# InternRobotics/InternNav

Measured on NVIDIA H100. Metric: InternVLA-N1 policy-steps/sec (batch RGB-D+text->action), higher is better.
Workload: dtype bf16

## Files before the change

internnav_b200/_lib.py:

```python
import ctypes
import os
import threading

import torch

_HERE = os.path.dirname(os.path.abspath(__file__))
LIB_PATH = os.path.join(_HERE, "libn1b200.so")

_lib = None
_lock = threading.Lock()

c_void_p, c_int, c_size_t, c_float, c_char_p = (
    ctypes.c_void_p, ctypes.c_int, ctypes.c_size_t, ctypes.c_float, ctypes.c_char_p)


class N1Error(RuntimeError):
    def __init__(self, code, msg):
        super().__init__("n1b200 error %d: %s" % (code, msg))
        self.code = code


class TensorDesc(ctypes.Structure):
    _fields_ = [("name", c_char_p), ("data", c_void_p), ("dtype", ctypes.c_int32), ("ndim", ctypes.c_int32),
                ("shape", ctypes.c_int64 * 4)]
# ... 85 lines not shown
    assert t.is_cuda and t.is_contiguous(), "n1b200 takes contiguous CUDA tensors"
    return c_void_p(t.data_ptr())


def stream_ptr():
    return c_void_p(torch.cuda.current_stream().cuda_stream)


def dtype_code(t):
    if t.dtype == torch.float32:
        return 0
    if t.dtype == torch.bfloat16:
        return 1
    raise TypeError("n1b200 takes fp32 or bf16 tensors, got %s" % t.dtype)


def prof_enable(on):
    lib().n1_prof_enable(1 if on else 0)


def prof_read():
    a, b = ctypes.c_double(), ctypes.c_double()
    c, d = ctypes.c_int64(), ctypes.c_int64()
    check(lib().n1_prof_read(ctypes.byref(a), ctypes.byref(b), ctypes.byref(c), ctypes.byref(d)))
    return {"gemm_ms": a.value, "gemm_flops": b.value, "gemm_launches": c.value, "total_launches": d.value}


def prof_read_shapes(cap=256):
    mnk = (ctypes.c_int32 * (3 * cap))()
    cnt = (ctypes.c_int64 * cap)()
    ms = (ctypes.c_double * cap)()
    n = lib().n1_prof_read_shapes(mnk, cnt, ms, cap)
    if n < 0:
        raise N1Error(n, lib().n1_last_error().decode("utf-8", "replace"))
    return [dict(M=mnk[3 * i], N=mnk[3 * i + 1], K=mnk[3 * i + 2], count=int(cnt[i]), ms=float(ms[i])) for i in range(n)]


def gemm(a, w, bias=None, gamma=None, residual=None, act=ACT_NONE, out_fp32=False, out=None):
    assert a.dtype == torch.bfloat16 and w.dtype == torch.bfloat16 and a.dim() == 2 and w.dim() == 2
    M, K = a.shape
    N = w.shape[0]
    n_out = N // 2 if act == ACT_SWIGLU else N
    if out is None:
        out = torch.empty(M, n_out, device=a.device, dtype=torch.float32 if out_fp32 else torch.bfloat16)
    assert a.stride(1) == 1 and w.stride(1) == 1 and out.stride(1) == 1
    check(lib().n1_op_gemm(c_void_p(a.data_ptr()), a.stride(0), c_void_p(w.data_ptr()), w.stride(0),
                           c_void_p(out.data_ptr()), out.stride(0), M, N, K, ptr(bias), ptr(gamma),
                           c_void_p(residual.data_ptr()) if residual is not None else None,
                           residual.stride(0) if residual is not None else 0, act, 1 if out_fp32 else 0, stream_ptr()))
    return out


def gemm_tile(a, w, out, bias=None, gamma=None, residual=None, act=ACT_NONE, rows_per_group=0, group_stride=0,
              group_offset=0, row_add=None, tile_n=0):
    fn = lib().n1_test_gemm
    fn.restype = c_int
    fn.argtypes = [c_void_p, c_int, c_void_p, c_int, c_void_p, c_int, c_int, c_int, c_int, c_void_p, c_void_p, c_void_p,
                   c_int, c_int, c_int, c_int, c_int, c_int, c_void_p, c_int, c_void_p]
    vp = lambda t: c_void_p(t.data_ptr()) if t is not None else None
    check(fn(vp(a), a.stride(0), vp(w), w.stride(0), vp(out), out.stride(0), a.shape[0], w.shape[0], a.shape[1],
             vp(bias), vp(gamma), vp(residual), residual.stride(0) if residual is not None else 0, act,
             1 if out.dtype == torch.float32 else 0, rows_per_group, group_stride, group_offset, vp(row_add), tile_n,
             stream_ptr()))
    return out


def layernorm(x, w, b=None, eps=1e-5, rms=False, out=None):
    assert x.dtype == torch.bfloat16 and x.dim() == 2 and x.stride(1) == 1
    y = torch.empty(x.shape, device=x.device, dtype=torch.bfloat16) if out is None else out
    assert y.stride(1) == 1 and y.shape == x.shape
    check(lib().n1_op_layernorm(c_void_p(x.data_ptr()), x.stride(0), c_void_p(y.data_ptr()), y.stride(0), ptr(w), ptr(b), x.shape[0],
                                x.shape[1], eps, 1 if rms else 0, stream_ptr()))
    return y


MOD_RMS_SCALE, MOD_LN_SCALE, MOD_GATED_RESIDUAL = 0, 1, 2


def mod_norm(x, w, mod, rows_per_group, eps, mode, residual=None, out=None):
    assert x.dtype == torch.bfloat16 and x.dim() == 2 and x.stride(1) == 1
    if out is None:
        out = torch.empty(x.shape, device=x.device, dtype=torch.bfloat16)
    if mod is not None:
        assert mod.dtype == torch.bfloat16 and mod.stride(1) == 1 and mod.shape[1] == x.shape[1]
        assert mod.shape[0] * rows_per_group == x.shape[0]
    check(lib().n1_op_mod_norm(c_void_p(x.data_ptr()), x.stride(0), ptr(w), c_void_p(mod.data_ptr()) if mod is not None else None,
                               mod.stride(0) if mod is not None else 0, int(rows_per_group),
                               c_void_p(residual.data_ptr()) if residual is not None else None,
                               residual.stride(0) if residual is not None else 0, c_void_p(out.data_ptr()), out.stride(0),
                               x.shape[0], x.shape[1], float(eps), int(mode), stream_ptr()))
    return out


def add(a, b, out=None):
    assert a.dtype == torch.bfloat16 and b.dtype == torch.bfloat16 and a.is_contiguous() and b.is_contiguous() and a.shape == b.shape
    if out is None:
        out = torch.empty_like(a)
    check(lib().n1_op_add(ptr(a), ptr(b), ptr(out), a.numel(), stream_ptr()))
    return out


def action_embed(lat, w, b, pos, out=None):
    assert lat.dtype == torch.float32 and lat.is_contiguous() and lat.shape[-1] == 3
    rows, (T, D) = lat.numel() // 3, pos.shape
    if out is None:
        out = torch.empty(rows, D, device=lat.device, dtype=torch.bfloat16)
    check(lib().n1_op_action_embed(ptr(lat), ptr(w), ptr(b), ptr(pos), ptr(out), rows, T, D, stream_ptr()))
    return out


def cfg_euler(pred, n, cfg, scale, dt, lat):
    assert pred.dtype == torch.bfloat16 and pred.stride(1) == 1 and lat.dtype == torch.float32 and lat.is_contiguous()
    assert pred.shape[0] == (2 if cfg else 1) * n and lat.numel() == 3 * n
    check(lib().n1_op_cfg_euler(c_void_p(pred.data_ptr()), pred.stride(0), n, 1 if cfg else 0, float(scale), float(dt), ptr(lat),
                                stream_ptr()))
    return lat

# ... 65 lines not shown
```

internnav_b200/csrc/api.cu:

```cuda
#include <string.h>

#include <string>
#include <vector>

#include "../../include/n1b200.h"
#include "n1_ops.h"
#include "resize.h"
#include "bwd_kernels.h"
#include "s1_model.h"
#include "s2_kernels.h"
#include "s2_model.h"
#include "weights.h"

using namespace n1;

struct n1_ctx {
  int device = 0;
  S1Model s1;
  S2Model s2;
};
struct n1_vit_plan_s {
  VitPlan* p;
};
struct n1_llm_plan_s {
// ... 698 lines not shown
    if (cu) memcpy(cu, v.cu_window.data(), v.cu_window.size() * sizeof(int32_t));
    if (n_cu) *n_cu = (int32_t)v.cu_window.size();
    if (pos_hw) memcpy(pos_hw, v.pos_hw.data(), v.pos_hw.size() * sizeof(int32_t));
  });
}

void n1_prof_enable(int on) { prof_enable(on != 0); }

void n1_prof_add(int64_t gemm_launches, int64_t total_launches) {
  prof_count_launch((int)(total_launches - gemm_launches));
  for (int64_t i = 0; i < gemm_launches; ++i) prof_count_gemm(0.0);
}

int n1_prof_read_shapes(int32_t* mnk, int64_t* count, double* ms, int cap) {
  int n = -1;
  guard([&] {
    if (!mnk || !count || !ms || cap <= 0) throw Error(N1_ERR_ARG, "n1_prof_read_shapes: bad arguments");
    n = prof_read_shapes(mnk, reinterpret_cast<long*>(count), ms, cap);
  });
  return n;
}

int n1_prof_read(double* gemm_ms, double* gemm_flops, int64_t* gemm_launches, int64_t* total_launches) {
  return guard([&] {
    ProfStats st = prof_read_and_reset();
    if (gemm_ms) *gemm_ms = st.gemm_ms;
    if (gemm_flops) *gemm_flops = st.gemm_flops;
    if (gemm_launches) *gemm_launches = st.gemm_launches;
    if (total_launches) *total_launches = st.total_launches;
  });
}

int n1_op_gemm(const void* A, int lda, const void* W, int ldw, void* out, int ldo, int M, int N, int K,
               const float* bias, const float* gamma, const void* residual, int ldr, int act, int out_fp32,
               void* stream) {
  return guard([&] {
    GemmEpilogue e;
    e.bias = bias, e.gamma = gamma, e.residual = B16(residual), e.ldr = ldr, e.act = act, e.out_fp32 = out_fp32;
    gemm_bf16(B16(A), lda, B16(W), ldw, out, ldo, M, N, K, e, S(stream));
  });
}

int n1_test_gemm(const void* A, int lda, const void* W, int ldw, void* out, int ldo, int M, int N, int K, const float* bias,
                 const float* gamma, const void* residual, int ldr, int act, int out_fp32, int rows_per_group,
                 int group_stride, int group_offset, const float* row_add, int tile_n, void* stream) {
  return guard([&] {
    GemmEpilogue e;
    e.bias = bias, e.gamma = gamma, e.residual = B16(residual), e.ldr = ldr, e.act = act, e.out_fp32 = out_fp32;
    e.rows_per_group = rows_per_group, e.group_stride = group_stride, e.group_offset = group_offset, e.row_add = row_add;
    gemm_bf16(B16(A), lda, B16(W), ldw, out, ldo, M, N, K, e, S(stream), tile_n);
  });
}

int n1_op_ff_block(const void* x, int ldx, const float* ln_w, const float* ln_b, float eps, const void* w1, const float* b1,
                   const void* w2, const float* b2, void* out, int ldo, int M, void* stream) {
  return guard([&] {
    ff_block_384(B16(x), ldx, ln_w, ln_b, eps, B16(w1), b1, B16(w2), b2, B16(out), ldo, M, S(stream));
  });
}

int n1_op_dec_sa_block(void* x, int ldx, const float* ln_w, const float* ln_b, float eps, const void* w_qkv,
                       const float* b_qkv, const void* w_o, const float* b_o, int B, int Ns, int T, int causal, void* stream) {
  return guard([&] {
    dec_sa_block(B16(x), ldx, ln_w, ln_b, eps, B16(w_qkv), b_qkv, B16(w_o), b_o, B, Ns, T, causal, S(stream));
  });
}
int n1_op_dec_ca_block(void* x, int ldx, const float* ln_w, const float* ln_b, float eps, const void* w_q, const float* b_q,
                       const void* w_o, const float* b_o, const void* kv, int ldkv, int mtok, int B, int Ns, int T,
                       void* stream) {
  return guard([&] {
    dec_ca_block(B16(x), ldx, ln_w, ln_b, eps, B16(w_q), b_q, B16(w_o), b_o, B16(kv), ldkv, mtok, B, Ns, T, S(stream));
  });
}

int n1_op_mod_norm(const void* x, int ldx, const float* w, const void* mod, int ld_mod, int rows_per_group, const void* res,
                   int ldr, void* out, int ldo, int64_t rows, int D, float eps, int mode, void* stream) {
  return guard([&] {
    mod_norm(B16(x), ldx, w, B16(mod), ld_mod, rows_per_group, B16(res), ldr, B16(out), ldo, rows, D, eps, mode, S(stream));
  });
}
int n1_op_add(const void* a, const void* b, void* out, int64_t n, void* stream) {
  return guard([&] { add_bf16(B16(a), B16(b), B16(out), n, S(stream)); });
}
int n1_op_action_embed(const float* lat, const float* w, const float* b, const float* pos, void* out, int64_t rows, int T, int D,
                       void* stream) {
  return guard([&] { action_embed(lat, w, b, pos, B16(out), rows, T, D, S(stream)); });
}
int n1_op_cfg_euler(const void* pred, int ld, int64_t n, int cfg, float scale, float dt, float* lat, void* stream) {
  return guard([&] { cfg_euler(B16(pred), ld, n, cfg, scale, dt, lat, S(stream)); });
}
int n1_op_layernorm(const void* x, int ldx, void* y, int ldy, const float* w, const float* b, int rows, int D, float eps,
                    int rms, void* stream) {
  return guard([&] { layernorm(B16(x), ldx, B16(y), ldy, w, b, rows, D, eps, rms, S(stream)); });
}

int n1_op_attention(const void* q, const void* k, const void* v, void* o, int ldq, int ldk, int ldv, int ldo, int heads_q,
                    int heads_kv, int head_dim, int batch, int seq_q, int seq_k, const int32_t* cu_q,
                    const int32_t* cu_k, int max_seq_q, int kv_div, int causal, float scale, void* stream) {
  return guard([&] {
    AttnParams p = {};
    p.q = B16(q), p.k = B16(k), p.v = B16(v), p.o = B16(o);
    p.ldq = ldq, p.ldk = ldk, p.ldv = ldv, p.ldo = ldo;
    p.heads_q = heads_q, p.heads_kv = heads_kv, p.hd = head_dim, p.batch = batch;
    p.seq_q = seq_q, p.seq_k = seq_k, p.cu_q = cu_q, p.cu_k = cu_k, p.max_seq_q = max_seq_q;
    p.kv_div = kv_div < 1 ? 1 : kv_div, p.causal = causal, p.scale = scale;
    attention(p, S(stream));
// ... 33 lines not shown
```

internnav_b200/csrc/gemm_wgmma.cu:

```cuda
#include <stdlib.h>

#include <algorithm>
#include <atomic>
#include <mutex>
#include <vector>

#include "n1_ops.h"
#include "n1_ptx.cuh"

namespace n1 {

namespace {

constexpr int BM = 128;
constexpr int BK = 64;
constexpr int kConsumerWarps = 8;
constexpr int kThreads = 32 * kConsumerWarps + 128;

template <int BN>
struct Cfg {
  static constexpr int kABytes = BM * BK * 2;
  static constexpr int kBBytes = BN * BK * 2;
  static constexpr int kStageBytes = kABytes + kBBytes;
  static constexpr int kStages = BN == 256 ? 4 : BN == 128 ? 6 : 8;
  static constexpr int kBarBytes = 256;
  static constexpr int kStoreBytes = kConsumerWarps * 2 * 1024;
  static constexpr int kSmemBytes = kStages * kStageBytes + kBarBytes + kStoreBytes + 1024;
};
static_assert(Cfg<256>::kSmemBytes <= 232448 && Cfg<128>::kSmemBytes <= 232448 && Cfg<64>::kSmemBytes <= 232448,
              "GEMM shared memory budget (227 KB per block)");

constexpr long kWStreamsBytes = 32L << 20;

struct GemmArgs {
  int M, N, K;
  int tiles_m, tiles_n;
  void* out;
  int ldo;
  const float* bias;
  const float* gamma;
  const bf16* residual;
  int ldr;
  int act;
  int out_fp32;
  int rows_per_group, group_stride, group_offset;
  const float* row_add;
  int raster_g;
  int tma_store;
};

__device__ __forceinline__ void decode_tile(int tile, int tiles_m, int tiles_n, int G, int& tm, int& tn) {
  const int per_group = G * tiles_n;
  const int g = tile / per_group;
  const int first_m = g * G;
  const int gsize = min(G, tiles_m - first_m);
  const int r = tile - g * per_group;
  tm = first_m + r % gsize;
  tn = r / gsize;
}

__device__ __forceinline__ float apply_act(float v, int act) {
  if (act == ACT_GELU) return gelu_erf(v);
  if (act == ACT_RELU) return fmaxf(v, 0.0f);
  if (act == ACT_GELU_TANH)
    return 0.5f * v * (1.0f + tanhf(0.7978845608028654f * (v + 0.044715f * v * v * v)));
  if (act == ACT_SILU) return silu(v);
  return v;
}

template <int BN>
__global__ void __launch_bounds__(kThreads, 1)
gemm_kernel(const __grid_constant__ CUtensorMap tmA, const __grid_constant__ CUtensorMap tmB,
            const __grid_constant__ CUtensorMap tmC, const GemmArgs args) {
  using C = Cfg<BN>;
  extern __shared__ uint8_t smem_raw[];
  uint8_t* smem = reinterpret_cast<uint8_t*>((reinterpret_cast<uintptr_t>(smem_raw) + 1023) & ~uintptr_t(1023));
  uint8_t* sA = smem;
  uint8_t* sB = smem + C::kStages * C::kABytes;
  uint64_t* bars = reinterpret_cast<uint64_t*>(smem + C::kStages * C::kStageBytes);
  uint64_t* full = bars;
  uint64_t* empty = bars + C::kStages;
  uint8_t* sStore = smem + C::kStages * C::kStageBytes + C::kBarBytes;

  const int warp = threadIdx.x >> 5;
  const int lane = threadIdx.x & 31;
  const int num_tiles = args.tiles_m * args.tiles_n;
  const int nkb = (args.K + BK - 1) / BK;

  if (threadIdx.x == 0) {
    tma_prefetch_desc(&tmA);
    tma_prefetch_desc(&tmB);
    if (args.tma_store) tma_prefetch_desc(&tmC);
    for (int s = 0; s < C::kStages; ++s) {
      mbar_init(&full[s], 1);
      mbar_init(&empty[s], kConsumerWarps);
    }
    fence_mbar_init();
  }
  __syncthreads();

  if (warp >= kConsumerWarps) {
    setmaxnreg_dec<kProducerRegs>();
    if (warp == kConsumerWarps && lane == 0) {
      int stage = 0;
      uint32_t phase = 0;
      for (int tile = blockIdx.x; tile < num_tiles; tile += gridDim.x) {
        int tm, tn;
        decode_tile(tile, args.tiles_m, args.tiles_n, args.raster_g, tm, tn);
        for (int kb = 0; kb < nkb; ++kb) {
          mbar_wait(&empty[stage], phase ^ 1);
          mbar_arrive_expect_tx(&full[stage], C::kStageBytes);
          tma_load_2d(sA + stage * C::kABytes, &tmA, &full[stage], kb * BK, tm * BM);
          tma_load_2d(sB + stage * C::kBBytes, &tmB, &full[stage], kb * BK, tn * BN);
          if (++stage == C::kStages) {
            stage = 0;
            phase ^= 1;
          }
        }
      }
    }
  } else {
    setmaxnreg_inc<kConsumerRegs>();
    const int wg = warp >> 2;
    const int wrow = wg * 64 + (warp & 3) * 16;
    const int quad = lane & 3;
    const bool swiglu = args.act == ACT_SWIGLU;
    uint8_t* my_store = sStore + warp * 2048;
    int sbuf = 0;
    int stage = 0;
    uint32_t phase = 0;
    for (int tile = blockIdx.x; tile < num_tiles; tile += gridDim.x) {
      int tm, tn;
      decode_tile(tile, args.tiles_m, args.tiles_n, args.raster_g, tm, tn);
      float acc[BN / 2];
      int prev = -1;
      for (int kb = 0; kb < nkb; ++kb) {
        mbar_wait(&full[stage], phase);
        const uint64_t adesc = wgmma_desc_sw128(smem_u32(sA + stage * C::kABytes + wg * 64 * 128));
        const uint64_t bdesc = wgmma_desc_sw128(smem_u32(sB + stage * C::kBBytes));
        wgmma_fence();
#pragma unroll
        for (int k = 0; k < BK / 16; ++k)
          wgmma_ss<0, 0>(acc, adesc + 2 * k, bdesc + 2 * k, (kb | k) != 0 ? 1u : 0u);
        wgmma_commit();
        wgmma_wait<1>();
        if (prev >= 0 && lane == 0) mbar_arrive(&empty[prev]);
        prev = stage;
        if (++stage == C::kStages) {
          stage = 0;
          phase ^= 1;
        }
      }
      wgmma_wait<0>();
      if (prev >= 0 && lane == 0) mbar_arrive(&empty[prev]);

      int row[2];
      long out_row[2];
      int grp_row[2] = {0, 0};
      bool row_ok[2];
#pragma unroll
      for (int h = 0; h < 2; ++h) {
        row[h] = tm * BM + wrow + (lane >> 2) + h * 8;
        row_ok[h] = row[h] < args.M;
        out_row[h] = row[h];
        if (args.rows_per_group > 0) {
          grp_row[h] = row[h] % args.rows_per_group;
          out_row[h] = (long)(row[h] / args.rows_per_group) * args.group_stride + grp_row[h] + args.group_offset;
        }
      }
#pragma unroll
      for (int chunk = 0; chunk < BN / 32; ++chunk) {
        const int col0 = tn * BN + chunk * 32;
        if (col0 >= args.N) break;
        float v[4][4];
#pragma unroll
        for (int j = 0; j < 4; ++j) {
          const int col = col0 + j * 8 + quad * 2;
          const bool col_ok = col < args.N;
#pragma unroll
          for (int e = 0; e < 4; ++e) v[j][e] = acc[(chunk * 4 + j) * 4 + e];
          if (args.bias && col_ok) {
            const float2 b = __ldg(reinterpret_cast<const float2*>(args.bias + col));
            v[j][0] += b.x, v[j][1] += b.y, v[j][2] += b.x, v[j][3] += b.y;
          }
          if (swiglu) {
            v[j][0] = silu(v[j][0]) * v[j][1];
            v[j][2] = silu(v[j][2]) * v[j][3];
            continue;
          }
#pragma unroll
          for (int e = 0; e < 4; ++e) v[j][e] = apply_act(v[j][e], args.act);
          if (args.gamma && col_ok) {
            const float2 g = __ldg(reinterpret_cast<const float2*>(args.gamma + col));
            v[j][0] *= g.x, v[j][1] *= g.y, v[j][2] *= g.x, v[j][3] *= g.y;
          }
#pragma unroll
          for (int h = 0; h < 2; ++h) {
            if (!row_ok[h] || !col_ok) continue;
            if (args.row_add) {
              const float2 a = __ldg(reinterpret_cast<const float2*>(args.row_add + (long)grp_row[h] * args.N + col));
              v[j][2 * h] += a.x, v[j][2 * h + 1] += a.y;
            }
            if (args.residual) {
              const uint32_t q = __ldg(reinterpret_cast<const uint32_t*>(args.residual + out_row[h] * args.ldr + col));
              v[j][2 * h] += bf16_lo(q), v[j][2 * h + 1] += bf16_hi(q);
            }
          }
        }
        if (args.tma_store) {
          if (lane == 0) tma_store_wait_read<1>();
          __syncwarp();
          uint8_t* sb = my_store + sbuf * 1024;
#pragma unroll
          for (int j = 0; j < 4; ++j)
#pragma unroll
            for (int h = 0; h < 2; ++h) {
              const int r = (lane >> 2) + h * 8;
              if (swiglu)
                *reinterpret_cast<bf16*>(sb + r * 32 + (j * 4 + quad) * 2) = __float2bfloat16_rn(v[j][2 * h]);
              else
                *reinterpret_cast<uint32_t*>(sb + r * 64 + (j * 8 + quad * 2) * 2) = pack_bf16(v[j][2 * h], v[j][2 * h + 1]);
            }
          fence_proxy_async_smem();
          __syncwarp();
          if (lane == 0) {
            tma_store_2d(&tmC, sb, swiglu ? col0 >> 1 : col0, tm * BM + wrow);
            tma_store_commit();
          }
          sbuf ^= 1;
          continue;
        }
#pragma unroll
        for (int j = 0; j < 4; ++j) {
          const int col = col0 + j * 8 + quad * 2;
          if (col >= args.N) continue;
#pragma unroll
          for (int h = 0; h < 2; ++h) {
            if (!row_ok[h]) continue;
            if (swiglu)
              reinterpret_cast<bf16*>(args.out)[out_row[h] * args.ldo + (col >> 1)] = __float2bfloat16_rn(v[j][2 * h]);
            else if (args.out_fp32)
              *reinterpret_cast<float2*>(reinterpret_cast<float*>(args.out) + out_row[h] * args.ldo + col) =
                  make_float2(v[j][2 * h], v[j][2 * h + 1]);
            else
              *reinterpret_cast<uint32_t*>(reinterpret_cast<bf16*>(args.out) + out_row[h] * args.ldo + col) =
                  pack_bf16(v[j][2 * h], v[j][2 * h + 1]);
          }
        }
      }
    }
    if (args.tma_store && lane == 0) tma_store_wait<0>();
    __syncwarp();
  }
}

typedef CUresult (*EncodeTiledFn)(CUtensorMap*, CUtensorMapDataType, cuuint32_t, void*, const cuuint64_t*,
                                  const cuuint64_t*, const cuuint32_t*, const cuuint32_t*, CUtensorMapInterleave,
                                  CUtensorMapSwizzle, CUtensorMapL2promotion, CUtensorMapFloatOOBfill);

EncodeTiledFn encode_fn() {
  static EncodeTiledFn fn = nullptr;
  static std::once_flag once;
  std::call_once(once, [] {
    void* p = nullptr;
    cudaDriverEntryPointQueryResult q;
    cudaError_t e = cudaGetDriverEntryPoint("cuTensorMapEncodeTiled", &p, cudaEnableDefault, &q);
    if (e == cudaSuccess && q == cudaDriverEntryPointSuccess) fn = reinterpret_cast<EncodeTiledFn>(p);
  });
  if (!fn) throw Error(-4, "cuTensorMapEncodeTiled unavailable (no CUDA driver / GPU?)");
  return fn;
}

CUtensorMap make_map(const bf16* ptr, long rows, long cols, long ld, int box_rows, int box_cols = BK, bool swizzle = true) {
  N1_CHECK((reinterpret_cast<uintptr_t>(ptr) & 15) == 0, "GEMM operand not 16-byte aligned");
  N1_CHECK(ld % 8 == 0, "GEMM operand leading dimension must be a multiple of 8 elements");
  CUtensorMap m;
  cuuint64_t gdim[2] = {(cuuint64_t)cols, (cuuint64_t)rows};
  cuuint64_t gstr[1] = {(cuuint64_t)ld * 2};
  cuuint32_t box[2] = {(cuuint32_t)box_cols, (cuuint32_t)box_rows};
  cuuint32_t estr[2] = {1, 1};
  CUresult r = encode_fn()(&m, CU_TENSOR_MAP_DATA_TYPE_BFLOAT16, 2, const_cast<bf16*>(ptr), gdim, gstr, box, estr,
                           CU_TENSOR_MAP_INTERLEAVE_NONE, swizzle ? CU_TENSOR_MAP_SWIZZLE_128B : CU_TENSOR_MAP_SWIZZLE_NONE,
                           CU_TENSOR_MAP_L2_PROMOTION_L2_256B, CU_TENSOR_MAP_FLOAT_OOB_FILL_NONE);
  if (r != CUDA_SUCCESS) throw Error(-5, "cuTensorMapEncodeTiled failed: " + std::to_string((int)r));
  return m;
}

template <int BN>
void launch(const bf16* A, int lda, const bf16* W, int ldw, int M, int N, int K, GemmArgs& a, cudaStream_t stream) {
  using C = Cfg<BN>;
  static std::once_flag once;
  std::call_once(once, [] {
    cudaFuncSetAttribute(gemm_kernel<BN>, cudaFuncAttributeMaxDynamicSharedMemorySize, C::kSmemBytes);
  });
  a.tiles_m = (M + BM - 1) / BM;
  a.tiles_n = (N + BN - 1) / BN;
  {
    const long panel = (long)BM * K * 2;
    const long w_bytes = (long)N * K * 2;
    int g = 8;
    if (w_bytes > kWStreamsBytes) g = (int)std::max<long>(2, (16L << 20) / panel);
    a.raster_g = g < a.tiles_m ? g : a.tiles_m;
    if (a.raster_g < 1) a.raster_g = 1;
  }
  CUtensorMap tmA = make_map(A, M, K, lda, BM);
  CUtensorMap tmB = make_map(W, N, K, ldw, BN);
  CUtensorMap tmC = tmA;
  if (a.tma_store) {
    const bool sw = a.act == ACT_SWIGLU;
    tmC = make_map(static_cast<const bf16*>(a.out), M, sw ? N / 2 : N, a.ldo, 16, sw ? 16 : 32, false);
  }
  const int tiles = a.tiles_m * a.tiles_n;
  const int grid = tiles < device_sm_count() ? tiles : device_sm_count();
  gemm_kernel<BN><<<grid, kThreads, C::kSmemBytes, stream>>>(tmA, tmB, tmC, a);
  N1_CUDA(cudaGetLastError());
}

std::atomic<long> g_total_launches{0}, g_gemm_launches{0};
std::atomic<bool> g_prof_on{false};
std::mutex g_prof_mu;
struct EvPair {
  cudaEvent_t a, b;
  double flops;
  int M, N, K;
};
std::vector<EvPair> g_events;
struct ShapeAcc {
  int M, N, K;
  long count;
  double ms;
};
std::vector<ShapeAcc> g_shapes;

}

CUtensorMap tma_map_2d(const bf16* ptr, long rows, long cols, long ld, int box_rows, int box_cols, bool swizzle) {
  return make_map(ptr, rows, cols, ld, box_rows, box_cols, swizzle);
}
CUtensorMap tma_map_3d_sw128(const bf16* ptr, const long dims[3], const long strides[2], const int box[3]) {
  N1_CHECK((reinterpret_cast<uintptr_t>(ptr) & 15) == 0 && strides[0] % 8 == 0 && strides[1] % 8 == 0,
           "tma_map_3d_sw128: 16-byte alignment");
  CUtensorMap m;
  cuuint64_t gdim[3] = {(cuuint64_t)dims[0], (cuuint64_t)dims[1], (cuuint64_t)dims[2]};
  cuuint64_t gstr[2] = {(cuuint64_t)strides[0] * 2, (cuuint64_t)strides[1] * 2};
  cuuint32_t bx[3] = {(cuuint32_t)box[0], (cuuint32_t)box[1], (cuuint32_t)box[2]};
  cuuint32_t estr[3] = {1, 1, 1};
  CUresult r = encode_fn()(&m, CU_TENSOR_MAP_DATA_TYPE_BFLOAT16, 3, const_cast<bf16*>(ptr), gdim, gstr, bx, estr,
                           CU_TENSOR_MAP_INTERLEAVE_NONE, CU_TENSOR_MAP_SWIZZLE_128B, CU_TENSOR_MAP_L2_PROMOTION_L2_256B,
                           CU_TENSOR_MAP_FLOAT_OOB_FILL_NONE);
  if (r != CUDA_SUCCESS) throw Error(-5, "cuTensorMapEncodeTiled (3-D) failed: " + std::to_string((int)r));
  return m;
}
void prof_count_gemm(double flops) {
  (void)flops;
  g_gemm_launches++;
  g_total_launches++;
}

void prof_enable(bool on) { g_prof_on = on; }
int prof_begin(double flops, int M, int N, int K, cudaStream_t s) {
  if (!g_prof_on.load()) return -1;
  EvPair ev{};
  cudaEventCreate(&ev.a);
  cudaEventCreate(&ev.b);
  ev.flops = flops, ev.M = M, ev.N = N, ev.K = K;
  cudaEventRecord(ev.a, s);
  std::lock_guard<std::mutex> lk(g_prof_mu);
// ... 5 lines not shown
  std::lock_guard<std::mutex> lk(g_prof_mu);
  if (ticket < (int)g_events.size()) cudaEventRecord(g_events[ticket].b, s);
}
void prof_count_launch(int n) { g_total_launches += n; }
ProfStats prof_read_and_reset() {
  ProfStats st;
  std::lock_guard<std::mutex> lk(g_prof_mu);
  for (EvPair& e : g_events) {
    cudaEventSynchronize(e.b);
    float ms = 0.f;
    if (cudaEventElapsedTime(&ms, e.a, e.b) == cudaSuccess) {
      st.gemm_ms += ms, st.gemm_flops += e.flops;
      bool hit = false;
      for (ShapeAcc& sa : g_shapes)
        if (sa.M == e.M && sa.N == e.N && sa.K == e.K) {
          sa.count++, sa.ms += ms, hit = true;
          break;
        }
      if (!hit) g_shapes.push_back({e.M, e.N, e.K, 1, (double)ms});
    }
    cudaEventDestroy(e.a);
    cudaEventDestroy(e.b);
  }
  g_events.clear();
  st.gemm_launches = g_gemm_launches.exchange(0);
  st.total_launches = g_total_launches.exchange(0);
  return st;
}

int prof_read_shapes(int* mnk, long* count, double* ms, int cap) {
  std::lock_guard<std::mutex> lk(g_prof_mu);
  int n = 0;
  for (const ShapeAcc& sa : g_shapes) {
    if (n >= cap) break;
    mnk[3 * n] = sa.M, mnk[3 * n + 1] = sa.N, mnk[3 * n + 2] = sa.K;
    count[n] = sa.count, ms[n] = sa.ms;
    ++n;
  }
  g_shapes.clear();
  return n;
}

int device_sm_count() {
  static int sms = 0;
  if (!sms) {
    int dev = 0;
    cudaGetDevice(&dev);
    cudaDeviceGetAttribute(&sms, cudaDevAttrMultiProcessorCount, dev);
    if (sms <= 0) sms = 132;
  }
  return sms;
}

void gemm_bf16(const bf16* A, int lda, const bf16* W, int ldw, void* out, int ldo, int M, int N, int K,
               const GemmEpilogue& e, cudaStream_t stream, int tile_n) {
  if (M <= 0 || N <= 0) return;
  N1_CHECK(tile_n == 0 || tile_n == 64 || tile_n == 128 || tile_n == 256, "GEMM tile width must be 0, 64, 128 or 256");
  N1_CHECK(K > 0 && K % 8 == 0, "GEMM K must be a positive multiple of 8");
  N1_CHECK(N % 8 == 0, "GEMM N must be a multiple of 8 (pad the packed weight)");
  N1_CHECK(!(e.act == ACT_SWIGLU) || N % 16 == 0, "SwiGLU GEMM needs N % 16 == 0");
  GemmArgs a;
  a.M = M, a.N = N, a.K = K;
  a.out = out, a.ldo = ldo;
  a.bias = e.bias, a.gamma = e.gamma, a.residual = e.residual, a.ldr = e.ldr;
  a.act = e.act, a.out_fp32 = e.out_fp32;
  a.rows_per_group = e.rows_per_group, a.group_stride = e.group_stride, a.group_offset = e.group_offset;
  a.row_add = e.row_add;
  a.tma_store = (!e.out_fp32 && e.rows_per_group == 0 && (reinterpret_cast<uintptr_t>(out) & 15) == 0 && ldo % 8 == 0) ? 1 : 0;
  const int sms = device_sm_count();
  const int tm = (M + BM - 1) / BM;
  auto cost = [&](int bn) {
    const long tiles = (long)tm * ((N + bn - 1) / bn);
    const long waves = (tiles + sms - 1) / sms;
    return waves * (bn + 48);
  };
  int bn = tile_n;
  if (bn == 0) {
    bn = cost(128) <= cost(64) ? 128 : 64;
    if ((long)N * K * 2 > kWStreamsBytes && cost(256) <= cost(bn)) bn = 256;
  }
  const double flops = 2.0 * M * (double)N * K;
  const int ticket = prof_begin(flops, M, N, K, stream);
  prof_count_gemm(flops);
  if (bn == 256) launch<256>(A, lda, W, ldw, M, N, K, a, stream);
  else if (bn == 128) launch<128>(A, lda, W, ldw, M, N, K, a, stream);
  else launch<64>(A, lda, W, ldw, M, N, K, a, stream);
  prof_end(ticket, stream);
}

}
```

internnav_b200/csrc/n1_ops.h:

```cpp
#pragma once
#include <cuda.h>
#include <cuda_bf16.h>
#include <cuda_runtime.h>
#include <stdint.h>

#include <stdexcept>
#include <string>

namespace n1 {

typedef __nv_bfloat16 bf16;

struct Error : std::runtime_error {
  int code;
  Error(int c, const std::string& m) : std::runtime_error(m), code(c) {}
};

#define N1_CHECK(cond, msg)                                                                       \
  do {                                                                                            \
    if (!(cond)) throw ::n1::Error(-2, std::string(__FILE__) + ":" + std::to_string(__LINE__) + \
                                           ": " + (msg));                                         \
  } while (0)

#define N1_CUDA(call)                                                                              \
  do {                                                                                             \
    cudaError_t e__ = (call);                                                                      \
    if (e__ != cudaSuccess)                                                                        \
      throw ::n1::Error(-3, std::string(__FILE__) + ":" + std::to_string(__LINE__) + ": " + #call + \
                                ": " + cudaGetErrorString(e__));                                   \
  } while (0)

enum GemmAct { ACT_NONE = 0, ACT_GELU = 1, ACT_RELU = 2, ACT_SWIGLU = 3, ACT_GELU_TANH = 4, ACT_SILU = 5 };

struct GemmEpilogue {
  const float* bias = nullptr;
  const float* gamma = nullptr;
  const bf16* residual = nullptr;
  int ldr = 0;
  int act = ACT_NONE;
  int out_fp32 = 0;
  int rows_per_group = 0, group_stride = 0, group_offset = 0;
  const float* row_add = nullptr;
};

void gemm_bf16(const bf16* A, int lda, const bf16* W, int ldw, void* out, int ldo, int M, int N, int K,
               const GemmEpilogue& epi, cudaStream_t stream, int tile_n = 0);

int device_sm_count();

CUtensorMap tma_map_2d(const bf16* ptr, long rows, long cols, long ld, int box_rows, int box_cols, bool swizzle);
CUtensorMap tma_map_3d_sw128(const bf16* ptr, const long dims[3], const long strides[2], const int box[3]);
void prof_count_gemm(double flops);

struct ProfStats {
  double gemm_ms = 0, gemm_flops = 0;
  long gemm_launches = 0, total_launches = 0;
};
void prof_enable(bool on);
void prof_count_launch(int n = 1);
int prof_begin(double flops, int M, int N, int K, cudaStream_t s);
void prof_end(int ticket, cudaStream_t s);
ProfStats prof_read_and_reset();
int prof_read_shapes(int* mnk, long* count, double* ms, int cap);

void layernorm(const bf16* x, int ldx, bf16* y, int ldy, const float* w, const float* b, int rows, int D,
               float eps, int rms, cudaStream_t stream);

struct AttnParams {
  const bf16* q;
  const bf16* k;
  const bf16* v;
  bf16* o;
  int ldq, ldk, ldv, ldo;
  int heads_q, heads_kv, hd;
  int batch;
  int seq_q, seq_k;
  const int* cu_q;
  const int* cu_k;
  int kv_div;
  int causal;
  float scale;
  int max_seq_q;
  const int* k_len;
  int k_slot;
  long total_rows;
  const int* k_row0;
};
void attention(const AttnParams& p, cudaStream_t stream);
bool attention_tc_supported(const AttnParams& p);
bool attention_uses_tc(const AttnParams& p);
void attention_tc128(const AttnParams& p, cudaStream_t stream);

struct CacheAttnParams {
  const bf16* q;
  int ldq;
  long q_rows;
  const bf16 *k, *v;
  int ldkv;
  long kv_rows;
// ... 28 lines not shown
```

Before: 66.65.

## Add ping-pong warpgroup GEMM schedule for 128-wide tiles with multiple waves

Adds a ping-pong WGMMA kernel where the two consumer warpgroups take alternate 128x128 tiles, ordered by mbarriers, so one warpgroup's epilogue overlaps the other's MMA main loop. The heuristic selects it automatically when the 128-wide tile is chosen and the tile count exceeds the SM count. The producer and epilogue are factored into shared helpers, and the epilogue is rolled for the 128-register accumulator. The cost is higher register pressure per consumer and extra barrier handshakes between warpgroups.

```diff
diff --git a/internnav_b200/_lib.py b/internnav_b200/_lib.py
--- a/internnav_b200/_lib.py
+++ b/internnav_b200/_lib.py
@@ -161,17 +161,43 @@
 
 
 def gemm_tile(a, w, out, bias=None, gamma=None, residual=None, act=ACT_NONE, rows_per_group=0, group_stride=0,
-              group_offset=0, row_add=None, tile_n=0):
-    fn = lib().n1_test_gemm
+              group_offset=0, row_add=None, tile_n=0, schedule=None):
+    assert schedule in (None, "pingpong"), schedule
+    assert schedule is None or tile_n == 0, "the ping-pong schedule has one tile width"
+    vp = lambda t: c_void_p(t.data_ptr()) if t is not None else None
+    args = [vp(a), a.stride(0), vp(w), w.stride(0), vp(out), out.stride(0), a.shape[0], w.shape[0], a.shape[1],
+            vp(bias), vp(gamma), vp(residual), residual.stride(0) if residual is not None else 0, act,
+            1 if out.dtype == torch.float32 else 0, rows_per_group, group_stride, group_offset, vp(row_add)]
+    types = [c_void_p, c_int, c_void_p, c_int, c_void_p, c_int, c_int, c_int, c_int, c_void_p, c_void_p, c_void_p,
+             c_int, c_int, c_int, c_int, c_int, c_int, c_void_p]
+    if schedule == "pingpong":
+        fn = lib().n1_test_gemm_pingpong
+    else:
+        fn = lib().n1_test_gemm
+        args.append(tile_n)
+        types.append(c_int)
     fn.restype = c_int
-    fn.argtypes = [c_void_p, c_int, c_void_p, c_int, c_void_p, c_int, c_int, c_int, c_int, c_void_p, c_void_p, c_void_p,
-                   c_int, c_int, c_int, c_int, c_int, c_int, c_void_p, c_int, c_void_p]
-    vp = lambda t: c_void_p(t.data_ptr()) if t is not None else None
-    check(fn(vp(a), a.stride(0), vp(w), w.stride(0), vp(out), out.stride(0), a.shape[0], w.shape[0], a.shape[1],
-             vp(bias), vp(gamma), vp(residual), residual.stride(0) if residual is not None else 0, act,
-             1 if out.dtype == torch.float32 else 0, rows_per_group, group_stride, group_offset, vp(row_add), tile_n,
-             stream_ptr()))
-    return out
+    fn.argtypes = types + [c_void_p]
+    check(fn(*args, stream_ptr()))
+    return out
+
+
+def gemm_choice(M, N, K, sms):
+    fn = lib().n1_test_gemm_choice
+    fn.restype = c_int
+    fn.argtypes = [c_int, c_int, c_int, c_int, ctypes.POINTER(ctypes.c_int32), ctypes.POINTER(ctypes.c_int32)]
+    t, p = ctypes.c_int32(), ctypes.c_int32()
+    check(fn(M, N, K, sms, ctypes.byref(t), ctypes.byref(p)))
+    return t.value, bool(p.value)
+
+
+def gemm_pingpong_start(wg, j, cta, grid, nkb):
+    fn = lib().n1_test_gemm_pingpong_start
+    fn.restype = c_int
+    fn.argtypes = [c_int, c_int, c_int, c_int, c_int, ctypes.POINTER(ctypes.c_int32)]
+    out = (ctypes.c_int32 * 4)()
+    check(fn(wg, j, cta, grid, nkb, out))
+    return tuple(out)
 
 
 def layernorm(x, w, b=None, eps=1e-5, rms=False, out=None):
diff --git a/internnav_b200/csrc/api.cu b/internnav_b200/csrc/api.cu
--- a/internnav_b200/csrc/api.cu
+++ b/internnav_b200/csrc/api.cu
@@ -774,6 +774,34 @@
   });
 }
 
+int n1_test_gemm_pingpong(const void* A, int lda, const void* W, int ldw, void* out, int ldo, int M, int N, int K,
+                          const float* bias, const float* gamma, const void* residual, int ldr, int act, int out_fp32,
+                          int rows_per_group, int group_stride, int group_offset, const float* row_add, void* stream) {
+  return guard([&] {
+    GemmEpilogue e;
+    e.bias = bias, e.gamma = gamma, e.residual = B16(residual), e.ldr = ldr, e.act = act, e.out_fp32 = out_fp32;
+    e.rows_per_group = rows_per_group, e.group_stride = group_stride, e.group_offset = group_offset, e.row_add = row_add;
+    gemm_bf16(B16(A), lda, B16(W), ldw, out, ldo, M, N, K, e, S(stream), 0, true);
+  });
+}
+int n1_test_gemm_choice(int M, int N, int K, int sms, int32_t* tile_n, int32_t* pingpong) {
+  return guard([&] {
+    if (M <= 0 || N <= 0 || K <= 0 || sms <= 0 || !tile_n || !pingpong)
+      throw Error(N1_ERR_ARG, "n1_test_gemm_choice: bad arguments");
+    const GemmChoice c = gemm_choice(M, N, K, sms);
+    *tile_n = c.tile_n, *pingpong = c.pingpong ? 1 : 0;
+  });
+}
+int n1_test_gemm_pingpong_start(int wg, int j, int cta, int grid, int nkb, int32_t* out4) {
+  return guard([&] {
+    if (wg < 0 || wg > 1 || j < 0 || cta < 0 || grid <= cta || nkb <= 0 || !out4)
+      throw Error(N1_ERR_ARG, "n1_test_gemm_pingpong_start: bad arguments");
+    const int stages = gemm_pingpong_stages();
+    const PingPongStart st = pingpong_start(wg, j, cta, grid, nkb, stages);
+    out4[0] = st.tile, out4[1] = st.stage, out4[2] = (int32_t)st.phase, out4[3] = stages;
+  });
+}
+
 int n1_op_ff_block(const void* x, int ldx, const float* ln_w, const float* ln_b, float eps, const void* w1, const float* b1,
                    const void* w2, const float* b2, void* out, int ldo, int M, void* stream) {
   return guard([&] {
diff --git a/internnav_b200/csrc/gemm_wgmma.cu b/internnav_b200/csrc/gemm_wgmma.cu
--- a/internnav_b200/csrc/gemm_wgmma.cu
+++ b/internnav_b200/csrc/gemm_wgmma.cu
@@ -27,6 +27,7 @@
   static constexpr int kStoreBytes = kConsumerWarps * 2 * 1024;
   static constexpr int kSmemBytes = kStages * kStageBytes + kBarBytes + kStoreBytes + 1024;
 };
+static_assert(2 * Cfg<128>::kStages + 2 <= Cfg<128>::kBarBytes / 8, "ping-pong barriers: full, empty, order");
 static_assert(Cfg<256>::kSmemBytes <= 232448 && Cfg<128>::kSmemBytes <= 232448 && Cfg<64>::kSmemBytes <= 232448,
               "GEMM shared memory budget (227 KB per block)");
 
@@ -69,6 +70,148 @@
 }
 
 template <int BN>
+__device__ __forceinline__ void produce(const CUtensorMap* tmA, const CUtensorMap* tmB, const GemmArgs& args, uint8_t* sA,
+                                        uint8_t* sB, uint64_t* full, uint64_t* empty, int num_tiles, int nkb) {
+  using C = Cfg<BN>;
+  int stage = 0;
+  uint32_t phase = 0;
+  for (int tile = blockIdx.x; tile < num_tiles; tile += gridDim.x) {
+    int tm, tn;
+    decode_tile(tile, args.tiles_m, args.tiles_n, args.raster_g, tm, tn);
+    for (int kb = 0; kb < nkb; ++kb) {
+      mbar_wait(&empty[stage], phase ^ 1);
+      mbar_arrive_expect_tx(&full[stage], C::kStageBytes);
+      tma_load_2d(sA + stage * C::kABytes, tmA, &full[stage], kb * BK, tm * BM);
+      tma_load_2d(sB + stage * C::kBBytes, tmB, &full[stage], kb * BK, tn * BN);
+      if (++stage == C::kStages) {
+        stage = 0;
+        phase ^= 1;
+      }
+    }
+  }
+}
+
+__device__ __forceinline__ void epilogue_chunk(const float* a, const GemmArgs& args, const CUtensorMap* tmC, int tm,
+                                               int col0, int wrow, int lane, uint8_t* my_store, int& sbuf) {
+  const int quad = lane & 3;
+  const bool swiglu = args.act == ACT_SWIGLU;
+  int row[2];
+  long out_row[2];
+  int grp_row[2] = {0, 0};
+  bool row_ok[2];
+#pragma unroll
+  for (int h = 0; h < 2; ++h) {
+    row[h] = tm * BM + wrow + (lane >> 2) + h * 8;
+    row_ok[h] = row[h] < args.M;
+    out_row[h] = row[h];
+    if (args.rows_per_group > 0) {
+      grp_row[h] = row[h] % args.rows_per_group;
+      out_row[h] = (long)(row[h] / args.rows_per_group) * args.group_stride + grp_row[h] + args.group_offset;
+    }
+  }
+  {
+    float v[4][4];
+#pragma unroll
+    for (int j = 0; j < 4; ++j) {
+      const int col = col0 + j * 8 + quad * 2;
+      const bool col_ok = col < args.N;
+#pragma unroll
+      for (int e = 0; e < 4; ++e) v[j][e] = a[j * 4 + e];
+      if (args.bias && col_ok) {
+        const float2 b = __ldg(reinterpret_cast<const float2*>(args.bias + col));
+        v[j][0] += b.x, v[j][1] += b.y, v[j][2] += b.x, v[j][3] += b.y;
+      }
+      if (swiglu) {
+        v[j][0] = silu(v[j][0]) * v[j][1];
+        v[j][2] = silu(v[j][2]) * v[j][3];
+        continue;
+      }
+#pragma unroll
+      for (int e = 0; e < 4; ++e) v[j][e] = apply_act(v[j][e], args.act);
+      if (args.gamma && col_ok) {
+        const float2 g = __ldg(reinterpret_cast<const float2*>(args.gamma + col));
+        v[j][0] *= g.x, v[j][1] *= g.y, v[j][2] *= g.x, v[j][3] *= g.y;
+      }
+#pragma unroll
+      for (int h = 0; h < 2; ++h) {
+        if (!row_ok[h] || !col_ok) continue;
+        if (args.row_add) {
+          const float2 a = __ldg(reinterpret_cast<const float2*>(args.row_add + (long)grp_row[h] * args.N + col));
+          v[j][2 * h] += a.x, v[j][2 * h + 1] += a.y;
+        }
+        if (args.residual) {
+          const uint32_t q = __ldg(reinterpret_cast<const uint32_t*>(args.residual + out_row[h] * args.ldr + col));
+          v[j][2 * h] += bf16_lo(q), v[j][2 * h + 1] += bf16_hi(q);
+        }
+      }
+    }
+    if (args.tma_store) {
+      if (lane == 0) tma_store_wait_read<1>();
+      __syncwarp();
+      uint8_t* sb = my_store + sbuf * 1024;
+#pragma unroll
+      for (int j = 0; j < 4; ++j)
+#pragma unroll
+        for (int h = 0; h < 2; ++h) {
+          const int r = (lane >> 2) + h * 8;
+          if (swiglu)
+            *reinterpret_cast<bf16*>(sb + r * 32 + (j * 4 + quad) * 2) = __float2bfloat16_rn(v[j][2 * h]);
+          else
+            *reinterpret_cast<uint32_t*>(sb + r * 64 + (j * 8 + quad * 2) * 2) = pack_bf16(v[j][2 * h], v[j][2 * h + 1]);
+        }
+      fence_proxy_async_smem();
+      __syncwarp();
+      if (lane == 0) {
+        tma_store_2d(tmC, sb, swiglu ? col0 >> 1 : col0, tm * BM + wrow);
+        tma_store_commit();
+      }
+      sbuf ^= 1;
+      return;
+    }
+#pragma unroll
+    for (int j = 0; j < 4; ++j) {
+      const int col = col0 + j * 8 + quad * 2;
+      if (col >= args.N) continue;
+#pragma unroll
+      for (int h = 0; h < 2; ++h) {
+        if (!row_ok[h]) continue;
+        if (swiglu)
+          reinterpret_cast<bf16*>(args.out)[out_row[h] * args.ldo + (col >> 1)] = __float2bfloat16_rn(v[j][2 * h]);
+        else if (args.out_fp32)
+          *reinterpret_cast<float2*>(reinterpret_cast<float*>(args.out) + out_row[h] * args.ldo + col) =
+              make_float2(v[j][2 * h], v[j][2 * h + 1]);
+        else
+          *reinterpret_cast<uint32_t*>(reinterpret_cast<bf16*>(args.out) + out_row[h] * args.ldo + col) =
+              pack_bf16(v[j][2 * h], v[j][2 * h + 1]);
+      }
+    }
+  }
+}
+
+
+template <int NV, int BN, bool kRolled>
+__device__ __forceinline__ void epilogue(float (&acc)[NV], const GemmArgs& args, const CUtensorMap* tmC, int tm, int tn,
+                                         int wrow, int lane, uint8_t* my_store, int& sbuf) {
+  constexpr int kPerSlab = BN / 32;
+  if constexpr (kRolled) {
+#pragma unroll 1
+    for (int c = 0; c < NV / 16; ++c) {
+      const int col0 = tn * BN + (c % kPerSlab) * 32;
+      if (col0 < args.N)
+        epilogue_chunk(acc, args, tmC, tm, col0, wrow + (c / kPerSlab) * 64, lane, my_store, sbuf);
+#pragma unroll
+      for (int i = 0; i + 16 < NV; ++i) acc[i] = acc[i + 16];
+    }
+  } else {
+#pragma unroll
+    for (int c = 0; c < NV / 16; ++c) {
+      const int col0 = tn * BN + (c % kPerSlab) * 32;
+      if (col0 < args.N) epilogue_chunk(acc + 16 * c, args, tmC, tm, col0, wrow + (c / kPerSlab) * 64, lane, my_store, sbuf);
+    }
+  }
+}
+
+template <int BN>
 __global__ void __launch_bounds__(kThreads, 1)
 gemm_kernel(const __grid_constant__ CUtensorMap tmA, const __grid_constant__ CUtensorMap tmB,
             const __grid_constant__ CUtensorMap tmC, const GemmArgs args) {
@@ -101,30 +244,10 @@
 
   if (warp >= kConsumerWarps) {
     setmaxnreg_dec<kProducerRegs>();
-    if (warp == kConsumerWarps && lane == 0) {
-      int stage = 0;
-      uint32_t phase = 0;
-      for (int tile = blockIdx.x; tile < num_tiles; tile += gridDim.x) {
-        int tm, tn;
-        decode_tile(tile, args.tiles_m, args.tiles_n, args.raster_g, tm, tn);
-        for (int kb = 0; kb < nkb; ++kb) {
-          mbar_wait(&empty[stage], phase ^ 1);
-          mbar_arrive_expect_tx(&full[stage], C::kStageBytes);
-          tma_load_2d(sA + stage * C::kABytes, &tmA, &full[stage], kb * BK, tm * BM);
-          tma_load_2d(sB + stage * C::kBBytes, &tmB, &full[stage], kb * BK, tn * BN);
-          if (++stage == C::kStages) {
-            stage = 0;
-            phase ^= 1;
-          }
-        }
-      }
-    }
+    if (warp == kConsumerWarps && lane == 0) produce<BN>(&tmA, &tmB, args, sA, sB, full, empty, num_tiles, nkb);
   } else {
     setmaxnreg_inc<kConsumerRegs>();
     const int wg = warp >> 2;
-    const int wrow = wg * 64 + (warp & 3) * 16;
-    const int quad = lane & 3;
-    const bool swiglu = args.act == ACT_SWIGLU;
     uint8_t* my_store = sStore + warp * 2048;
     int sbuf = 0;
     int stage = 0;
@@ -153,101 +276,91 @@
       }
       wgmma_wait<0>();
       if (prev >= 0 && lane == 0) mbar_arrive(&empty[prev]);
-
-      int row[2];
-      long out_row[2];
-      int grp_row[2] = {0, 0};
-      bool row_ok[2];
-#pragma unroll
-      for (int h = 0; h < 2; ++h) {
-        row[h] = tm * BM + wrow + (lane >> 2) + h * 8;
-        row_ok[h] = row[h] < args.M;
-        out_row[h] = row[h];
-        if (args.rows_per_group > 0) {
-          grp_row[h] = row[h] % args.rows_per_group;
-          out_row[h] = (long)(row[h] / args.rows_per_group) * args.group_stride + grp_row[h] + args.group_offset;
-        }
-      }
-#pragma unroll
-      for (int chunk = 0; chunk < BN / 32; ++chunk) {
-        const int col0 = tn * BN + chunk * 32;
-        if (col0 >= args.N) break;
-        float v[4][4];
-#pragma unroll
-        for (int j = 0; j < 4; ++j) {
-          const int col = col0 + j * 8 + quad * 2;
-          const bool col_ok = col < args.N;
-#pragma unroll
-          for (int e = 0; e < 4; ++e) v[j][e] = acc[(chunk * 4 + j) * 4 + e];
-          if (args.bias && col_ok) {
-            const float2 b = __ldg(reinterpret_cast<const float2*>(args.bias + col));
-            v[j][0] += b.x, v[j][1] += b.y, v[j][2] += b.x, v[j][3] += b.y;
-          }
-          if (swiglu) {
-            v[j][0] = silu(v[j][0]) * v[j][1];
-            v[j][2] = silu(v[j][2]) * v[j][3];
-            continue;
-          }
-#pragma unroll
-          for (int e = 0; e < 4; ++e) v[j][e] = apply_act(v[j][e], args.act);
-          if (args.gamma && col_ok) {
-            const float2 g = __ldg(reinterpret_cast<const float2*>(args.gamma + col));
-            v[j][0] *= g.x, v[j][1] *= g.y, v[j][2] *= g.x, v[j][3] *= g.y;
-          }
-#pragma unroll
-          for (int h = 0; h < 2; ++h) {
-            if (!row_ok[h] || !col_ok) continue;
-            if (args.row_add) {
-              const float2 a = __ldg(reinterpret_cast<const float2*>(args.row_add + (long)grp_row[h] * args.N + col));
-              v[j][2 * h] += a.x, v[j][2 * h + 1] += a.y;
-            }
-            if (args.residual) {
-              const uint32_t q = __ldg(reinterpret_cast<const uint32_t*>(args.residual + out_row[h] * args.ldr + col));
-              v[j][2 * h] += bf16_lo(q), v[j][2 * h + 1] += bf16_hi(q);
-            }
-          }
-        }
-        if (args.tma_store) {
-          if (lane == 0) tma_store_wait_read<1>();
-          __syncwarp();
-          uint8_t* sb = my_store + sbuf * 1024;
-#pragma unroll
-          for (int j = 0; j < 4; ++j)
-#pragma unroll
-            for (int h = 0; h < 2; ++h) {
-              const int r = (lane >> 2) + h * 8;
-              if (swiglu)
-                *reinterpret_cast<bf16*>(sb + r * 32 + (j * 4 + quad) * 2) = __float2bfloat16_rn(v[j][2 * h]);
-              else
-                *reinterpret_cast<uint32_t*>(sb + r * 64 + (j * 8 + quad * 2) * 2) = pack_bf16(v[j][2 * h], v[j][2 * h + 1]);
-            }
-          fence_proxy_async_smem();
-          __syncwarp();
-          if (lane == 0) {
-            tma_store_2d(&tmC, sb, swiglu ? col0 >> 1 : col0, tm * BM + wrow);
-            tma_store_commit();
-          }
-          sbuf ^= 1;
-          continue;
-        }
-#pragma unroll
-        for (int j = 0; j < 4; ++j) {
-          const int col = col0 + j * 8 + quad * 2;
-          if (col >= args.N) continue;
-#pragma unroll
-          for (int h = 0; h < 2; ++h) {
-            if (!row_ok[h]) continue;
-            if (swiglu)
-              reinterpret_cast<bf16*>(args.out)[out_row[h] * args.ldo + (col >> 1)] = __float2bfloat16_rn(v[j][2 * h]);
-            else if (args.out_fp32)
-              *reinterpret_cast<float2*>(reinterpret_cast<float*>(args.out) + out_row[h] * args.ldo + col) =
-                  make_float2(v[j][2 * h], v[j][2 * h + 1]);
-            else
-              *reinterpret_cast<uint32_t*>(reinterpret_cast<bf16*>(args.out) + out_row[h] * args.ldo + col) =
-                  pack_bf16(v[j][2 * h], v[j][2 * h + 1]);
-          }
-        }
-      }
+      epilogue<BN / 2, BN, false>(acc, args, &tmC, tm, tn, wg * 64 + (warp & 3) * 16, lane, my_store, sbuf);
+    }
+    if (args.tma_store && lane == 0) tma_store_wait<0>();
+    __syncwarp();
+  }
+}
+
+__global__ void __launch_bounds__(kThreads, 1)
+gemm_pingpong(const __grid_constant__ CUtensorMap tmA, const __grid_constant__ CUtensorMap tmB,
+              const __grid_constant__ CUtensorMap tmC, const GemmArgs args) {
+  using C = Cfg<128>;
+  extern __shared__ uint8_t smem_raw[];
+  uint8_t* smem = reinterpret_cast<uint8_t*>((reinterpret_cast<uintptr_t>(smem_raw) + 1023) & ~uintptr_t(1023));
+  uint8_t* sA = smem;
+  uint8_t* sB = smem + C::kStages * C::kABytes;
+  uint64_t* bars = reinterpret_cast<uint64_t*>(smem + C::kStages * C::kStageBytes);
+  uint64_t* full = bars;
+  uint64_t* empty = bars + C::kStages;
+  uint64_t* order = bars + 2 * C::kStages;
+  uint8_t* sStore = smem + C::kStages * C::kStageBytes + C::kBarBytes;
+
+  const int warp = threadIdx.x >> 5;
+  const int lane = threadIdx.x & 31;
+  const int num_tiles = args.tiles_m * args.tiles_n;
+  const int nkb = (args.K + BK - 1) / BK;
+
+  if (threadIdx.x == 0) {
+    tma_prefetch_desc(&tmA);
+    tma_prefetch_desc(&tmB);
+    if (args.tma_store) tma_prefetch_desc(&tmC);
+    for (int s = 0; s < C::kStages; ++s) {
+      mbar_init(&full[s], 1);
+      mbar_init(&empty[s], kConsumerWarps / 2);
+    }
+    mbar_init(&order[0], kConsumerWarps / 2);
+    mbar_init(&order[1], kConsumerWarps / 2);
+    fence_mbar_init();
+  }
+  __syncthreads();
+
+  if (warp >= kConsumerWarps) {
+    setmaxnreg_dec<kProducerRegs>();
+    if (warp == kConsumerWarps && lane == 0) produce<128>(&tmA, &tmB, args, sA, sB, full, empty, num_tiles, nkb);
+  } else {
+    setmaxnreg_inc<kConsumerRegs>();
+    const int wg = warp >> 2;
+    uint8_t* my_store = sStore + warp * 2048;
+    int sbuf = 0;
+    for (int j = 0;; ++j) {
+      const PingPongStart st = pingpong_start(wg, j, blockIdx.x, gridDim.x, nkb, C::kStages);
+      if (st.tile >= num_tiles) break;
+      int tm, tn;
+      decode_tile(st.tile, args.tiles_m, args.tiles_n, args.raster_g, tm, tn);
+      if (wg == 1) mbar_wait(&order[0], j & 1);
+      else if (j > 0) mbar_wait(&order[1], (j - 1) & 1);
+      int stage = st.stage;
+      uint32_t phase = st.phase;
+      float acc[128];
+      float(&acc_lo)[64] = *reinterpret_cast<float(*)[64]>(acc);
+      float(&acc_hi)[64] = *reinterpret_cast<float(*)[64]>(acc + 64);
+      int prev = -1;
+      for (int kb = 0; kb < nkb; ++kb) {
+        mbar_wait(&full[stage], phase);
+        const uint64_t adesc0 = wgmma_desc_sw128(smem_u32(sA + stage * C::kABytes));
+        const uint64_t adesc1 = wgmma_desc_sw128(smem_u32(sA + stage * C::kABytes + 64 * 128));
+        const uint64_t bdesc = wgmma_desc_sw128(smem_u32(sB + stage * C::kBBytes));
+        wgmma_fence();
+#pragma unroll
+        for (int k = 0; k < BK / 16; ++k) {
+          wgmma_ss<0, 0>(acc_lo, adesc0 + 2 * k, bdesc + 2 * k, (kb | k) != 0 ? 1u : 0u);
+          wgmma_ss<0, 0>(acc_hi, adesc1 + 2 * k, bdesc + 2 * k, (kb | k) != 0 ? 1u : 0u);
+        }
+        wgmma_commit();
+        wgmma_wait<1>();
+        if (prev >= 0 && lane == 0) mbar_arrive(&empty[prev]);
+        prev = stage;
+        if (++stage == C::kStages) {
+          stage = 0;
+          phase ^= 1;
+        }
+      }
+      if (lane == 0) mbar_arrive(&order[wg]);
+      wgmma_wait<0>();
+      if (lane == 0) mbar_arrive(&empty[prev]);
+      epilogue<128, 128, true>(acc, args, &tmC, tm, tn, (warp & 3) * 16, lane, my_store, sbuf);
     }
     if (args.tma_store && lane == 0) tma_store_wait<0>();
     __syncwarp();
@@ -286,12 +399,14 @@
   return m;
 }
 
-template <int BN>
+template <int BN, bool kPingPong>
 void launch(const bf16* A, int lda, const bf16* W, int ldw, int M, int N, int K, GemmArgs& a, cudaStream_t stream) {
   using C = Cfg<BN>;
+  static_assert(!kPingPong || BN == 128, "the ping-pong schedule has 128 x 128 tiles");
+  const auto kernel = kPingPong ? gemm_pingpong : gemm_kernel<BN>;
   static std::once_flag once;
-  std::call_once(once, [] {
-    cudaFuncSetAttribute(gemm_kernel<BN>, cudaFuncAttributeMaxDynamicSharedMemorySize, C::kSmemBytes);
+  std::call_once(once, [kernel] {
+    cudaFuncSetAttribute(kernel, cudaFuncAttributeMaxDynamicSharedMemorySize, C::kSmemBytes);
   });
   a.tiles_m = (M + BM - 1) / BM;
   a.tiles_n = (N + BN - 1) / BN;
@@ -312,7 +427,7 @@
   }
   const int tiles = a.tiles_m * a.tiles_n;
   const int grid = tiles < device_sm_count() ? tiles : device_sm_count();
-  gemm_kernel<BN><<<grid, kThreads, C::kSmemBytes, stream>>>(tmA, tmB, tmC, a);
+  kernel<<<grid, kThreads, C::kSmemBytes, stream>>>(tmA, tmB, tmC, a);
   N1_CUDA(cudaGetLastError());
 }
 
@@ -424,10 +539,24 @@
   return sms;
 }
 
+int gemm_pingpong_stages() { return Cfg<128>::kStages; }
+
+GemmChoice gemm_choice(int M, int N, int K, int sms) {
+  const int tm = (M + BM - 1) / BM;
+  auto tiles = [&](int bn) { return (long)tm * ((N + bn - 1) / bn); };
+  auto cost = [&](int bn) { return (tiles(bn) + sms - 1) / sms * (bn + 48); };
+  GemmChoice c;
+  c.tile_n = cost(128) <= cost(64) ? 128 : 64;
+  if ((long)N * K * 2 > kWStreamsBytes && cost(256) <= cost(c.tile_n)) c.tile_n = 256;
+  c.pingpong = c.tile_n == 128 && tiles(128) > sms;
+  return c;
+}
+
 void gemm_bf16(const bf16* A, int lda, const bf16* W, int ldw, void* out, int ldo, int M, int N, int K,
-               const GemmEpilogue& e, cudaStream_t stream, int tile_n) {
+               const GemmEpilogue& e, cudaStream_t stream, int tile_n, bool pingpong) {
   if (M <= 0 || N <= 0) return;
   N1_CHECK(tile_n == 0 || tile_n == 64 || tile_n == 128 || tile_n == 256, "GEMM tile width must be 0, 64, 128 or 256");
+  N1_CHECK(!pingpong || tile_n == 0, "the ping-pong GEMM schedule has one tile width; pass tile_n = 0");
   N1_CHECK(K > 0 && K % 8 == 0, "GEMM K must be a positive multiple of 8");
   N1_CHECK(N % 8 == 0, "GEMM N must be a multiple of 8 (pad the packed weight)");
   N1_CHECK(!(e.act == ACT_SWIGLU) || N % 16 == 0, "SwiGLU GEMM needs N % 16 == 0");
@@ -439,24 +568,16 @@
   a.rows_per_group = e.rows_per_group, a.group_stride = e.group_stride, a.group_offset = e.group_offset;
   a.row_add = e.row_add;
   a.tma_store = (!e.out_fp32 && e.rows_per_group == 0 && (reinterpret_cast<uintptr_t>(out) & 15) == 0 && ldo % 8 == 0) ? 1 : 0;
-  const int sms = device_sm_count();
-  const int tm = (M + BM - 1) / BM;
-  auto cost = [&](int bn) {
-    const long tiles = (long)tm * ((N + bn - 1) / bn);
-    const long waves = (tiles + sms - 1) / sms;
-    return waves * (bn + 48);
-  };
-  int bn = tile_n;
-  if (bn == 0) {
-    bn = cost(128) <= cost(64) ? 128 : 64;
-    if ((long)N * K * 2 > kWStreamsBytes && cost(256) <= cost(bn)) bn = 256;
-  }
+  GemmChoice c{tile_n, pingpong};
+  if (tile_n == 0 && !pingpong) c = gemm_choice(M, N, K, device_sm_count());
+  if (c.pingpong) c.tile_n = 128;
   const double flops = 2.0 * M * (double)N * K;
   const int ticket = prof_begin(flops, M, N, K, stream);
   prof_count_gemm(flops);
-  if (bn == 256) launch<256>(A, lda, W, ldw, M, N, K, a, stream);
-  else if (bn == 128) launch<128>(A, lda, W, ldw, M, N, K, a, stream);
-  else launch<64>(A, lda, W, ldw, M, N, K, a, stream);
+  if (c.pingpong) launch<128, true>(A, lda, W, ldw, M, N, K, a, stream);
+  else if (c.tile_n == 256) launch<256, false>(A, lda, W, ldw, M, N, K, a, stream);
+  else if (c.tile_n == 128) launch<128, false>(A, lda, W, ldw, M, N, K, a, stream);
+  else launch<64, false>(A, lda, W, ldw, M, N, K, a, stream);
   prof_end(ticket, stream);
 }
 
diff --git a/internnav_b200/csrc/n1_ops.h b/internnav_b200/csrc/n1_ops.h
--- a/internnav_b200/csrc/n1_ops.h
+++ b/internnav_b200/csrc/n1_ops.h
@@ -44,7 +44,24 @@
 };
 
 void gemm_bf16(const bf16* A, int lda, const bf16* W, int ldw, void* out, int ldo, int M, int N, int K,
-               const GemmEpilogue& epi, cudaStream_t stream, int tile_n = 0);
+               const GemmEpilogue& epi, cudaStream_t stream, int tile_n = 0, bool pingpong = false);
+
+struct GemmChoice {
+  int tile_n;
+  bool pingpong;
+};
+GemmChoice gemm_choice(int M, int N, int K, int sms);
+
+struct PingPongStart {
+  int tile, stage;
+  uint32_t phase;
+};
+__host__ __device__ inline PingPongStart pingpong_start(int wg, int j, int cta, int grid, int nkb, int stages) {
+  const long t = 2L * j + wg;
+  const long pos = t * nkb;
+  return {cta + (int)t * grid, (int)(pos % stages), (uint32_t)((pos / stages) & 1)};
+}
+int gemm_pingpong_stages();
 
 int device_sm_count();
 
```

Measured after the change: 68.73 (median of 6 runs). 1.03x the previous value.
